# ducha-aiki/affnet

Measured on NVIDIA H100. Metric: Mpix/s end-to-end HesAffNet(+OriNet)+HardNet, higher is better.
Workload: dtype fp16 operands (fp16 residual planes: AffNet/OriNet weights+activations, HardNet layer 2-3 weights), fp32 accumulate; stencils fp32

## Files before the change

affnet_b200/csrc/nets_tcx.cu:

```cuda
#include <stdlib.h>
#include <string.h>

#include <vector>

#include <cuda_bf16.h>

#include "net_impl.cuh"
#include "tcx_conv.cuh"
#include "tcx_first.cuh"

namespace ag {
namespace tcx {

static int num_sms() {
    static int n = 0;
    if (n == 0) {
        int dev = 0;
        cudaGetDevice(&dev);
        cudaDeviceGetAttribute(&n, cudaDevAttrMultiProcessorCount, dev);
        if (n <= 0) n = 132;
    }
    return n;
}

static int ensure_smem_attr(const void* func, int bytes, bool* configured, const char* what) {
    int dev = 0;
    cudaGetDevice(&dev);
    dev &= 63;
    if (configured[dev]) return AG_OK;
    int rc = check_cuda(cudaFuncSetAttribute(func, cudaFuncAttributeMaxDynamicSharedMemorySize, bytes), what);
    if (rc == AG_OK) configured[dev] = true;
    return rc;
}

template <int CIN, int COUT, int H, int STRIDE, int NSPLIT, int STAGES, int OUT, int SA, int SW, int OSA, int BF = 0, int MC = 0>
static int launch_conv(const void* in, void* out, const __half* w, const float* b, float inv_scale, int n, int group, const int* count, cudaStream_t st) {
    using Cfg = XCfg<CIN, COUT, H, STRIDE, NSPLIT, STAGES, OUT, SA, SW, OSA>;
    auto kern = tcx_conv_kernel<CIN, COUT, H, STRIDE, NSPLIT, STAGES, OUT, SA, SW, OSA, BF, MC>;
    static bool configured[64] = {};
    int rc = ensure_smem_attr((const void*)kern, (int)Cfg::SMEM, configured, "tcx_conv smem attr");
    if (rc != AG_OK) return rc;
    XArgs a;
    a.in = (const __half*)in; a.out = out; a.wpk = w; a.bias = b; a.inv_scale = inv_scale; a.n = n; a.group = group; a.count = count;
    const int units = Cfg::In::PAIR ? (n + 1) / 2 : n;
    int gx = num_sms() / NSPLIT;
    if (gx > units) gx = units;
    if (gx < 1) gx = 1;
    if (MC) {
        cudaLaunchConfig_t cfg;
        memset(&cfg, 0, sizeof(cfg));
        cfg.gridDim = dim3(gx, NSPLIT); cfg.blockDim = dim3(Cfg::THREADS); cfg.dynamicSmemBytes = Cfg::SMEM; cfg.stream = st;
        cudaLaunchAttribute attr[1];
        attr[0].id = cudaLaunchAttributeClusterDimension;
        attr[0].val.clusterDim.x = 1; attr[0].val.clusterDim.y = 2; attr[0].val.clusterDim.z = 1;
        cfg.attrs = attr; cfg.numAttrs = 1;
        rc = check_cuda(cudaLaunchKernelEx(&cfg, kern, a), "tcx_conv cluster launch");
        if (rc != AG_OK) return rc;
    } else
        kern<<<dim3(gx, NSPLIT), Cfg::THREADS, Cfg::SMEM, st>>>(a);
    AG_CHECK_LAUNCH("tcx_conv_kernel");
    return AG_OK;
}

template <int C1, int COUT, int SA, int SW, int OSA, int BF = 0, int L3 = 0>
static int launch_first(void* out, const __half* w, const float* b, float inv_scale, int n, int group, const int* count, cudaStream_t st, const FirstSrc& src,
                        void* out3 = nullptr, const __half* w3 = nullptr, const float* b3 = nullptr, float inv_scale3 = 0.f) {
    using Cfg = XFirstCfg<C1, COUT, SA, SW, OSA, L3>;
    auto kern = tcx_first_kernel<C1, COUT, SA, SW, OSA, BF, L3>;
    static bool configured[64] = {};
    int rc = ensure_smem_attr((const void*)kern, (int)Cfg::SMEM, configured, "tcx_first smem attr");
    if (rc != AG_OK) return rc;
    XArgs a;
    a.in = nullptr; a.out = out; a.wpk = w; a.bias = b; a.inv_scale = inv_scale; a.n = n; a.group = group; a.count = count;
    XArgs a3 = a;
    a3.out = out3; a3.wpk = w3; a3.bias = b3; a3.inv_scale = inv_scale3;
    int gx = num_sms();
    if (gx > n) gx = n;
    if (gx < 1) gx = 1;
    kern<<<gx, Cfg::THREADS, Cfg::SMEM, st>>>(a, src, a3);
    AG_CHECK_LAUNCH("tcx_first_kernel");
    return AG_OK;
}

__global__ void tcx_decode_kernel(const __half* __restrict__ buf, int layout, int C, int osa, int H, int n, float* __restrict__ out) {
    const size_t total = (size_t)n * C * H * H;
    for (size_t i = (size_t)blockIdx.x * blockDim.x + threadIdx.x; i < total; i += (size_t)gridDim.x * blockDim.x) {
        const int x = (int)(i % H), y = (int)((i / H) % H), c = (int)((i / ((size_t)H * H)) % C), pi = (int)(i / ((size_t)H * H * C));
        const int slots = layout_slots(layout);
        const size_t unit_halfs = (size_t)(C / 8) * slots * 8 * (osa ? 2 : 1);
        const int unit = layout_pair(layout) ? (pi >> 1) : pi;
        const int slot = layout_slot(layout, y, x, pi & 1);
        const __half* ub = buf + (size_t)unit * unit_halfs;
        float v = __half2float(ub[((size_t)(c / 8) * slots + slot) * 8 + (c & 7)]);
        if (osa) v += __half2float(ub[((size_t)(C / 8 + c / 8) * slots + slot) * 8 + (c & 7)]);
        out[i] = v;
    }
}

}

static __half bf16_bits_as_half(float v) {
    const __nv_bfloat16 b = __float2bfloat16_rn(v);
    __half h;
    memcpy(&h, &b, 2);
    return h;
}
static float bf16_round(float v) { return __bfloat162float(__float2bfloat16_rn(v)); }

void tcx_pack_layer(const float* wf, int ci, int co, int stride, int nsplit, int sw, float scale, std::vector<__half>& out, int bf16) {
    const int nt = co / nsplit;
    auto put = [&](int dy, int dx, int cin, int c, int part) {
        const float v = scale * wf[((size_t)(dy * 3 + dx) * ci + cin) * co + c];
        if (bf16) {
            const float hi = bf16_round(v);
            out.push_back(bf16_bits_as_half(part == 0 ? hi : v - hi));
        } else {
            const __half hi = __float2half_rn(v);
            out.push_back(part == 0 ? hi : __float2half_rn(v - __half2float(hi)));
        }
    };
    for (int sp = 0; sp < nsplit; sp++)
        for (int dy = 0; dy < 3; dy++)
            for (int j = 0; j < ci / 16; j++) {
                if (stride == 1) {
                    for (int kg = 0; kg < 2; kg++)
                        for (int part = 0; part <= sw; part++)
                            for (int dx = 0; dx < 3; dx++)
                                for (int c = 0; c < nt; c++)
                                    for (int e = 0; e < 8; e++) put(dy, dx, (2 * j + kg) * 8 + e, sp * nt + c, part);
                } else {
                    for (int kg = 0; kg < 2; kg++)
                        for (int part = 0; part <= sw; part++)
                            for (int dx = 0; dx < 3; dx += 2)
                                for (int c = 0; c < nt; c++)
                                    for (int e = 0; e < 8; e++) put(dy, dx, (2 * j + kg) * 8 + e, sp * nt + c, part);
                    for (int kg = 0; kg < 2; kg++)
                        for (int part = 0; part <= sw; part++)
                            for (int c = 0; c < nt; c++)
                                for (int e = 0; e < 8; e++) put(dy, 1, (2 * j + kg) * 8 + e, sp * nt + c, part);
                }
            }
}

int tcx_nsplit(int kind, int layer) { return (kind == AG_NET_HARDNET && layer >= 4) ? 2 : 1; }
#ifndef AG_HARD_SW2
#define AG_HARD_SW2 1
#endif
#ifndef AG_HARD_SW3
#define AG_HARD_SW3 1
#endif
#ifndef AG_HARD_SW4
#define AG_HARD_SW4 0
#endif
int tcx_split_w(int kind, int layer) { return kind == AG_NET_HARDNET ? (layer == 1 ? AG_HARD_SW2 : layer == 2 ? AG_HARD_SW3 : layer == 3 ? AG_HARD_SW4 : 0) : 1; }
int tcx_stride(int layer) { return (layer == 2 || layer == 4) ? 2 : 1; }

size_t tcx_act_bytes(int n) { return (size_t)(n + 1) * 65536; }

#ifndef AG_HARD_MC5
#define AG_HARD_MC5 1
#endif
#ifndef AG_HARD_MC6
#define AG_HARD_MC6 0
#endif
int tcx_trunk_affori(const ag_net* net, const tc::FirstSrc& src0, int n, int group, const int* count, void* bufA, void* bufB, void* feat,
                     cudaStream_t st, int upto) {
    using namespace tcx;
    tc::FirstSrc src = src0;
    src.w1 = net->d_w1; src.b1 = net->d_b[0]; src.w1_inv = net->w_inv_scale[0]; src.w1_scale = 1.0f / net->w_inv_scale[0];
    int rc;
    if (upto <= 2) return launch_first<16, 16, 1, 1, 1>(bufB, net->d_wx[1], net->d_b[1], net->w_inv_scale[1], n, group, count, st, src);
    if ((rc = launch_first<16, 16, 1, 1, 1, 0, 1>(nullptr, net->d_wx[1], net->d_b[1], net->w_inv_scale[1], n, group, count, st, src,
                                                   bufA, net->d_wx[2], net->d_b[2], net->w_inv_scale[2]))) return rc;
    if (upto <= 3) return AG_OK;
    if ((rc = launch_conv<32, 32, 16, 1, 1, 4, L_S2_8P, 1, 1, 1>(bufA, bufB, net->d_wx[3], net->d_b[3], net->w_inv_scale[3], n, group, count, st))) return rc;
    if (upto <= 4) return AG_OK;
    if ((rc = launch_conv<32, 64, 16, 2, 1, 2, L_S1_8P, 1, 1, 1>(bufB, bufA, net->d_wx[4], net->d_b[4], net->w_inv_scale[4], n, group, count, st))) return rc;
    if (upto <= 5) return AG_OK;
    return launch_conv<64, 64, 8, 1, 1, 2, L_HEAD, 1, 1, 1>(bufA, feat, net->d_wx[5], net->d_b[5], net->w_inv_scale[5], n, group, count, st);
}

template <int BF>
static int trunk_hardnet_t(const ag_net* net, const tc::FirstSrc& src0, int n, int group, const int* count, void* bufA, void* bufB, void* headbuf,
                           cudaStream_t st, int upto) {
    using namespace tcx;
    tc::FirstSrc src = src0;
    src.w1 = net->d_w1; src.b1 = net->d_b[0]; src.w1_inv = net->w_inv_scale[0]; src.w1_scale = 1.0f / net->w_inv_scale[0];
    __half* const* wx = BF ? net->d_wx_bf : net->d_wx;
    int rc;
    if ((rc = launch_first<32, 32, 0, AG_HARD_SW2, 0, BF>(bufB, wx[1], net->d_b[1], net->w_inv_scale[1], n, group, count, st, src))) return rc;
    if (upto <= 2) return AG_OK;
    if ((rc = launch_conv<32, 64, 32, 2, 1, 2, L_S1_16, 0, AG_HARD_SW3, 0, BF>(bufB, bufA, wx[2], net->d_b[2], net->w_inv_scale[2], n, group, count, st))) return rc;
    if (upto <= 3) return AG_OK;
    if ((rc = launch_conv<64, 64, 16, 1, 1, 2, L_S2_8P, 0, AG_HARD_SW4, 0, BF>(bufA, bufB, wx[3], net->d_b[3], net->w_inv_scale[3], n, group, count, st))) return rc;
    if (upto <= 4) return AG_OK;
    if ((rc = launch_conv<64, 128, 16, 2, 2, 2, L_S1_8P, 0, 0, 0, BF, AG_HARD_MC5>(bufB, bufA, wx[4], net->d_b[4], net->w_inv_scale[4], n, group, count, st))) return rc;
    if (upto <= 5) return AG_OK;
    return launch_conv<128, 128, 8, 1, 2, 2, L_HEAD, 0, 0, 0, BF, AG_HARD_MC6>(bufA, headbuf, wx[5], net->d_b[5], net->w_inv_scale[5], n, group, count, st);
}

int tcx_trunk_hardnet(const ag_net* net, const tc::FirstSrc& src0, int n, int group, const int* count, void* bufA, void* bufB, void* headbuf,
                      cudaStream_t st, int upto, int bf16) {
    return bf16 ? trunk_hardnet_t<1>(net, src0, n, group, count, bufA, bufB, headbuf, st, upto)
                : trunk_hardnet_t<0>(net, src0, n, group, count, bufA, bufB, headbuf, st, upto);
}

}

using namespace ag;

extern "C" {

int ag_debug_tcx_layer(const ag_net_t* net, const float* d_patches, int n, int upto, float* d_out, void* d_ws, size_t ws_bytes, void* stream) {
    AG_REQUIRE(net && d_patches && d_out && d_ws, "NULL argument");
    AG_REQUIRE(upto >= 2 && upto <= 5 && n >= 1, "layer out of range");
    const size_t act = align_up(tcx_act_bytes(n), 256);
    AG_REQUIRE(ws_bytes >= 2 * act, "workspace too small");
    cudaStream_t st = (cudaStream_t)stream;
    char* base = (char*)d_ws;
    const tc::FirstSrc src = tc_src_patches(d_patches);
    const bool hard = net->kind == AG_NET_HARDNET;
    int rc = hard ? tcx_trunk_hardnet(net, src, n, n, nullptr, base, base + act, nullptr, st, upto)
                  : tcx_trunk_affori(net, src, n, n, nullptr, base, base + act, nullptr, st, upto);
    if (rc) return rc;
    const int lay = upto == 2 ? tcx::L_S2_16 : upto == 3 ? tcx::L_S1_16 : upto == 4 ? tcx::L_S2_8P : tcx::L_S1_8P;
    const int H = upto == 2 ? 32 : (upto <= 4 ? 16 : 8);
    const int Cb = hard ? 32 : 16;
    const int C = upto == 2 ? Cb : (upto <= 4 ? 2 * Cb : 4 * Cb);
    const void* buf = (upto == 2 || upto == 4) ? base + act : base;
    const int osa = hard ? 0 : 1;
    tcx::tcx_decode_kernel<<<296, 256, 0, st>>>((const __half*)buf, lay, C, osa, H, n, d_out);
    AG_CHECK_LAUNCH("tcx_decode_kernel");
    return AG_OK;
}

#ifdef AG_FIRST_TIMELINE
int ag_first_timeline_read(unsigned long long* host, int* dims, int reset) {
    constexpr size_t n = (size_t)tcx::TL_LAUNCHES * tcx::TL_CTAS * 16 * tcx::TL_STATES;
    if (dims) { dims[0] = tcx::TL_LAUNCHES; dims[1] = tcx::TL_CTAS; dims[2] = tcx::TL_STATES; }
    cudaDeviceSynchronize();
    if (host) {
        const int rc = check_cuda(cudaMemcpyFromSymbol(host, tcx::g_first_tl, n * 8), "timeline read");
        if (rc != AG_OK) return rc;
    }
    if (reset) {
        static unsigned long long zeros[n];
        static int zl[tcx::TL_CTAS];
        int rc = check_cuda(cudaMemcpyToSymbol(tcx::g_first_tl, zeros, sizeof(zeros)), "timeline reset");
        if (rc == AG_OK) rc = check_cuda(cudaMemcpyToSymbol(tcx::g_first_tl_launch, zl, sizeof(zl)), "timeline reset");
        return rc;
    }
    return AG_OK;
}
#endif

}
```

affnet_b200/csrc/tcx_conv.cuh:

```cuda
#pragma once
#include <cuda_bf16.h>

#include "tc_conv.cuh"

namespace ag {
namespace tcx {

using namespace ag::tc;

enum XLayout { L_S2_16 = 0, L_S1_16 = 1, L_S2_8P = 2, L_S1_8P = 3, L_HEAD = 4 };

__device__ __forceinline__ void bulk_g2s_mc(void* dst, const void* src, uint32_t bytes, uint64_t* bar, uint16_t mask) {
    asm volatile("cp.async.bulk.shared::cluster.global.mbarrier::complete_tx::bytes.multicast::cluster [%0], [%1], %2, [%3], %4;" ::"r"(smem_u32(dst)),
                 "l"(src), "r"(bytes), "r"(smem_u32(bar)), "h"(mask)
                 : "memory");
}
__device__ __forceinline__ void mbar_arrive_cluster(uint64_t* bar, uint32_t cta) {
    asm volatile("{\n .reg .b32 ra;\n mapa.shared::cluster.u32 ra, %0, %1;\n mbarrier.arrive.release.cluster.shared::cluster.b64 _, [ra];\n}\n" ::"r"(smem_u32(bar)), "r"(cta)
                 : "memory");
}
__device__ __forceinline__ void cluster_sync() {
    asm volatile("barrier.cluster.arrive.release.aligned;\n barrier.cluster.wait.acquire.aligned;" ::: "memory");
}

template <int BF>
__device__ __forceinline__ uint32_t pack2(float a, float b) {
    if (BF) { const __nv_bfloat162 h = __floats2bfloat162_rn(a, b); return *reinterpret_cast<const uint32_t*>(&h); }
    const __half2 h = __floats2half2_rn(a, b);
    return *reinterpret_cast<const uint32_t*>(&h);
}
template <int BF>
__device__ __forceinline__ float2 unpack2(uint32_t u) {
    if (BF) return make_float2(__uint_as_float(u << 16), __uint_as_float(u & 0xFFFF0000u));
    return __half22float2(*reinterpret_cast<const __half2*>(&u));
}
template <int LO, int BF = 0>
__device__ __forceinline__ void split_pack8(const float* v, uint4& hi, uint4& lo) {
    uint32_t h[4], l[4];
#pragma unroll
    for (int i = 0; i < 4; i++) {
        h[i] = pack2<BF>(v[2 * i], v[2 * i + 1]);
        if (LO) {
            const float2 f = unpack2<BF>(h[i]);
            l[i] = pack2<BF>(v[2 * i] - f.x, v[2 * i + 1] - f.y);
        } else l[i] = 0;
    }
    hi = make_uint4(h[0], h[1], h[2], h[3]);
    lo = make_uint4(l[0], l[1], l[2], l[3]);
}

template <int LO, int BF = 0>
__device__ __forceinline__ void split_pack2(float v0, float v1, uint32_t& hi, uint32_t& lo) {
    hi = pack2<BF>(v0, v1);
    if (LO) {
        const float2 f = unpack2<BF>(hi);
        lo = pack2<BF>(v0 - f.x, v1 - f.y);
    } else lo = 0;
}

__host__ __device__ constexpr int layout_slots(int lay) { return lay == L_S2_16 ? 1024 : lay == L_S1_16 ? 256 : lay == L_S2_8P ? 512 : 128; }
__host__ __device__ constexpr int layout_pair(int lay) { return (lay == L_S2_8P || lay == L_S1_8P) ? 1 : 0; }
__host__ __device__ constexpr int layout_slot(int lay, int y, int x, int p) {
    return lay == L_S2_16 ? ((y & 1) * 2 + (x & 1)) * 256 + (y >> 1) * 16 + (x >> 1)
         : lay == L_S1_16 ? y * 16 + x
         : lay == L_S2_8P ? ((y & 1) * 2 + (x & 1)) * 128 + ((y >> 1) * 2 + p) * 8 + (x >> 1)
                          : (y * 2 + p) * 8 + x;
}

template <int H, int STRIDE>
struct XIn {
    static constexpr int HOUT = H / STRIDE;
    static constexpr int PAIR = (HOUT == 8) ? 1 : 0;
    static constexpr int W = HOUT;
    static constexpr int RW = W * (1 + PAIR);
    static constexpr int TILES = HOUT * RW / 128;
    static constexpr int NPLANES = (STRIDE == 1) ? 1 : 4;
    static constexpr int DATA = HOUT * RW;
    static constexpr int PLANE = DATA + RW;
    static constexpr int SLOT_STAGE = NPLANES * PLANE;
    static constexpr int LAYOUT = (STRIDE == 2) ? (PAIR ? L_S2_8P : L_S2_16) : (PAIR ? L_S1_8P : L_S1_16);
    static_assert(HOUT == 8 || HOUT == 16 || HOUT == 32, "map sizes of the three nets");
    static_assert(!(STRIDE == 1 && H == 32), "the 32x32 stride-1 layer lives in tcx_first.cuh");
};

struct XArgs {
    const __half* in;
    void* out;
    const __half* wpk;
    const float* bias;
    float inv_scale;
    int n, group;
    const int* count;
};

template <int CIN, int COUT, int H, int STRIDE, int NSPLIT, int STAGES, int OUT, int SA, int SW, int OSA>
struct XCfg {
    using In = XIn<H, STRIDE>;
    static constexpr int CO = COUT, STRD = STRIDE, OUTL = OUT, SPLIT_A = SA, SPLIT_W = SW, SPLIT_O = OSA;
    static constexpr int KC = CIN / 8, NT = COUT / NSPLIT, HOUT = In::HOUT;
    static constexpr int G = KC * (1 + SA);
    static constexpr int GS = STAGES * In::SLOT_STAGE + (STRIDE == 1 ? In::RW : 0);
    static constexpr int ACCW = 3 * NT;
    static constexpr int BLOCKS = 2 * In::TILES;
    static constexpr uint32_t W_BYTES = 9u * CIN * NT * 2u * (1 + SW);
    static constexpr uint32_t IN_BYTES = (uint32_t)G * GS * 16u;
    static constexpr uint32_t HI_IN_BYTES = (uint32_t)KC * In::NPLANES * In::DATA * 16u;
    static constexpr uint32_t UNIT_IN_BYTES = HI_IN_BYTES * (1 + SA);
    static constexpr int THREADS = 288;
    static constexpr size_t SMEM = 1024 + (size_t)W_BYTES + IN_BYTES;
    static constexpr size_t HI_OUT_BYTES = (size_t)(COUT / 8) * layout_slots(OUT) * 16;
    static constexpr size_t UNIT_OUT_BYTES = (OUT == L_HEAD) ? 0 : HI_OUT_BYTES * (1 + OSA);
    static constexpr int NR1 = (1 + SW) * 3 * NT;
    static constexpr int NRO = (1 + SW) * 2 * NT, NRE = (1 + SW) * NT;
    static_assert(CIN % 16 == 0 && NT % 16 == 0 && ACCW <= 256, "wgmma shape");
    static_assert(In::W == 8 || In::W == 16, "a warp's 16 accumulator rows hold whole image rows");
    static_assert(SA <= 1 && SW <= 1 && OSA <= 1, "split-precision switches are 0 | 1");
    static_assert(2 * STAGES + 1 <= 60, "barrier area");
    static_assert(SMEM <= 232448, "shared memory budget");
    static_assert(GS < 16384, "leading-byte offset field");
    static_assert(OUT == L_HEAD || layout_pair(OUT) || !In::PAIR, "a pair layer writes pair layouts or the head operand");
};

__device__ __forceinline__ void frag_left(float v0, float v1, int lane, float& l0, float& l1) {
    const float s0 = __shfl_sync(0xffffffffu, v0, (lane + 28) & 31), s1 = __shfl_sync(0xffffffffu, v1, (lane + 28) & 31);
    l0 = s0;
    l1 = lane < 4 ? s0 : s1;
}
__device__ __forceinline__ void frag_right(float v0, float v1, int lane, float& r0, float& r1) {
    const float t0 = __shfl_sync(0xffffffffu, v0, (lane + 4) & 31), t1 = __shfl_sync(0xffffffffu, v1, (lane + 4) & 31);
    r0 = lane >= 28 ? t1 : t0;
    r1 = t1;
}

__device__ __forceinline__ bool xpatch_valid(const XArgs& a, int pi) { return pi < a.n && (a.count == nullptr || (pi % a.group) < a.count[pi / a.group]); }

template <class Cfg, int BF>
__device__ __forceinline__ void xconv_block_issue(float* d, uint32_t a_t, uint32_t w_base) {
    using In = typename Cfg::In;
    constexpr int KC = Cfg::KC, NT = Cfg::NT, GS = Cfg::GS, RW = In::RW, SA = Cfg::SPLIT_A, SW = Cfg::SPLIT_W;
    constexpr uint32_t LBO_A = ((uint32_t)GS) << 16;
    wgmma_fence();
    if (Cfg::STRD == 1) {
#pragma unroll
        for (int dy = 0; dy < 3; dy++) {
#pragma unroll
            for (int j = 0; j < KC / 2; j++) {
                const uint32_t ahi = ((a_t + (uint32_t)(dy * RW + 2 * j * GS)) & 0x3FFFu) | LBO_A;
                const uint32_t alo = ((a_t + (uint32_t)(dy * RW + (KC + 2 * j) * GS)) & 0x3FFFu) | LBO_A;
                const uint32_t blk = w_base + (uint32_t)((dy * (KC / 2) + j) * 2 * Cfg::NR1);
                const uint32_t bhi = (blk & 0x3FFFu) | ((uint32_t)Cfg::NR1 << 16), blo = ((blk + 3 * NT) & 0x3FFFu) | ((uint32_t)Cfg::NR1 << 16);
                Wgmma<3 * NT, BF>::mma(d, desc64(ahi), desc64(bhi), (dy | j) != 0);
                if (SW) Wgmma<3 * NT, BF>::mma(d, desc64(ahi), desc64(blo), 1);
                if (SA) Wgmma<3 * NT, BF>::mma(d, desc64(alo), desc64(bhi), 1);
            }
        }
    } else {
#pragma unroll
        for (int dy = 0; dy < 3; dy++) {
            constexpr int PL = In::PLANE;
            const int py = (dy == 1) ? 0 : 1, ro = (dy == 0) ? 0 : 1;
#pragma unroll
            for (int j = 0; j < KC / 2; j++) {
                const uint32_t blk = w_base + (uint32_t)((dy * (KC / 2) + j) * 2 * (Cfg::NRO + Cfg::NRE));
                const uint32_t bo_hi = (blk & 0x3FFFu) | ((uint32_t)Cfg::NRO << 16), bo_lo = ((blk + 2 * NT) & 0x3FFFu) | ((uint32_t)Cfg::NRO << 16);
                const uint32_t be = blk + 2 * Cfg::NRO;
                const uint32_t be_hi = (be & 0x3FFFu) | ((uint32_t)Cfg::NRE << 16), be_lo = ((be + NT) & 0x3FFFu) | ((uint32_t)Cfg::NRE << 16);
                const uint32_t ao = a_t + (uint32_t)((py * 2 + 1) * PL + ro * RW);
                const uint32_t ao_hi = ((ao + (uint32_t)(2 * j * GS)) & 0x3FFFu) | LBO_A, ao_lo = ((ao + (uint32_t)((KC + 2 * j) * GS)) & 0x3FFFu) | LBO_A;
                Wgmma<2 * NT, BF>::mma(d, desc64(ao_hi), desc64(bo_hi), (dy | j) != 0);
                if (SW) Wgmma<2 * NT, BF>::mma(d, desc64(ao_hi), desc64(bo_lo), 1);
                if (SA) Wgmma<2 * NT, BF>::mma(d, desc64(ao_lo), desc64(bo_hi), 1);
                const uint32_t ae = a_t + (uint32_t)((py * 2 + 0) * PL + ro * RW);
                const uint32_t ae_hi = ((ae + (uint32_t)(2 * j * GS)) & 0x3FFFu) | LBO_A, ae_lo = ((ae + (uint32_t)((KC + 2 * j) * GS)) & 0x3FFFu) | LBO_A;
                Wgmma<NT, BF>::mma(d + NT, desc64(ae_hi), desc64(be_hi), (dy | j) != 0);
                if (SW) Wgmma<NT, BF>::mma(d + NT, desc64(ae_hi), desc64(be_lo), 1);
                if (SA) Wgmma<NT, BF>::mma(d + NT, desc64(ae_lo), desc64(be_hi), 1);
            }
        }
    }
    wgmma_commit();
}
template <class Cfg, int BF>
__device__ __forceinline__ void xconv_block_mma(float* d, uint32_t a_t, uint32_t w_base) {
    xconv_block_issue<Cfg, BF>(d, a_t, w_base);
    wgmma_wait<0>();
    wgmma_reg_fence<Cfg::ACCW / 2>(d);
}

template <class Cfg, int BF>
__device__ __forceinline__ void xconv_block_epilogue(const float* d, const XArgs& a, const float* s_bias, int u, int b, int split, int wq, int lane) {
    using In = typename Cfg::In;
    constexpr int NT = Cfg::NT, HOUT = Cfg::HOUT, W = In::W, PAIR = In::PAIR, COUT = Cfg::CO, OUT = Cfg::OUTL, OSA = Cfg::SPLIT_O;
    unsigned char* obase[2];
    bool has_l[2], has_r[2];
    bool ok[2];
    size_t lo_off = 0;
#pragma unroll
    for (int h = 0; h < 2; h++) {
        const int r = b * 64 + wq * 16 + (lane >> 2) + 8 * h;
        int y, x, pi;
        if (PAIR) { y = r >> 4; x = r & 7; pi = 2 * u + ((r >> 3) & 1); }
        else { y = r / W; x = r - y * W; pi = u; }
        ok[h] = xpatch_valid(a, pi);
        has_l[h] = x > 0; has_r[h] = x < W - 1;
        if (OUT == L_HEAD) {
            obase[h] = reinterpret_cast<unsigned char*>(a.out) + (((size_t)(pi >> 7) * (HOUT * HOUT * COUT / 8) + (size_t)(y * HOUT + x) * (COUT / 8)) * 128 + (pi & 127)) * 16;
            lo_off = (size_t)((a.n + 127) >> 7) * (HOUT * HOUT * COUT / 8) * 128 * 16;
        } else {
            const int ou = layout_pair(OUT) ? (pi >> 1) : pi;
            obase[h] = reinterpret_cast<unsigned char*>(a.out) + (size_t)ou * Cfg::UNIT_OUT_BYTES + (size_t)layout_slot(OUT, y, x, pi & 1) * 16;
            lo_off = (size_t)(COUT / 8) * layout_slots(OUT) * 16;
        }
    }
#pragma unroll
    for (int j = 0; j < NT / 8; j++) {
        const int c = j * 8 + 2 * (lane & 3);
        float v[2][2];
#pragma unroll
        for (int e = 0; e < 2; e++) {
            const float c00 = d[4 * j + e], c01 = d[4 * j + 2 + e];
            const float c10 = d[4 * (j + NT / 8) + e], c11 = d[4 * (j + NT / 8) + 2 + e];
            const float c20 = d[4 * (j + 2 * NT / 8) + e], c21 = d[4 * (j + 2 * NT / 8) + 2 + e];
            float l0, l1;
            frag_left(c00, c01, lane, l0, l1);
            float acc0, acc1;
            if (Cfg::STRD == 1) {
                float r0, r1;
                frag_right(c20, c21, lane, r0, r1);
                const float t0 = has_r[0] ? r0 + c10 : c10, t1 = has_r[1] ? r1 + c11 : c11;
                acc0 = has_l[0] ? l0 + t0 : t0;
                acc1 = has_l[1] ? l1 + t1 : t1;
            } else {
                const float t0 = c10 + c20, t1 = c11 + c21;
                acc0 = has_l[0] ? l0 + t0 : t0;
                acc1 = has_l[1] ? l1 + t1 : t1;
            }
            v[0][e] = fmaxf(fmaf(acc0, a.inv_scale, s_bias[c + e]), 0.f);
            v[1][e] = fmaxf(fmaf(acc1, a.inv_scale, s_bias[c + e]), 0.f);
        }
        const int ch = split * NT + c;
        const size_t goff = ((OUT == L_HEAD) ? (size_t)(ch / 8) * 128 * 16 : (size_t)(ch / 8) * layout_slots(OUT) * 16) + (ch & 7) * 2;
#pragma unroll
        for (int h = 0; h < 2; h++) {
            if (!ok[h]) continue;
            uint32_t hi, lo;
            split_pack2<OSA, BF>(v[h][0], v[h][1], hi, lo);
            *reinterpret_cast<uint32_t*>(obase[h] + goff) = hi;
            if (OSA) *reinterpret_cast<uint32_t*>(obase[h] + lo_off + goff) = lo;
        }
    }
}

template <int CIN, int COUT, int H, int STRIDE, int NSPLIT, int STAGES, int OUT, int SA, int SW, int OSA, int BF = 0, int MC = 0>
__global__ void __launch_bounds__(288, 1) tcx_conv_kernel(const XArgs a) {
    static_assert(MC == 0 || NSPLIT == 2, "multicast pairs the two channel-split CTAs");
    using Cfg = XCfg<CIN, COUT, H, STRIDE, NSPLIT, STAGES, OUT, SA, SW, OSA>;
    using In = typename Cfg::In;
    constexpr int ACCW = Cfg::ACCW, BLOCKS = Cfg::BLOCKS, GS = Cfg::GS, RW = In::RW;
    constexpr int PAIR = In::PAIR;
    extern __shared__ __align__(1024) unsigned char smem[];
    uint64_t* full = reinterpret_cast<uint64_t*>(smem);
    uint64_t* empty = full + STAGES;
    uint64_t* wbar = empty + STAGES;
    float* s_bias = reinterpret_cast<float*>(smem + 512);
    unsigned char* sW = smem + 1024;
    unsigned char* sIn = sW + Cfg::W_BYTES;

    const int warp = threadIdx.x >> 5, lane = threadIdx.x & 31;
    const int split = blockIdx.y;
    const int n_units = PAIR ? (a.n + 1) >> 1 : a.n;

    if (threadIdx.x < Cfg::NT) s_bias[threadIdx.x] = a.bias[split * Cfg::NT + threadIdx.x];
    if (threadIdx.x == 0) {
        for (int s = 0; s < STAGES; s++) { mbar_init(&full[s], 1); mbar_init(&empty[s], 2 * (1 + MC)); }
        mbar_init(wbar, 1);
        asm volatile("fence.mbarrier_init.release.cluster;" ::: "memory");
    }
    for (int i = threadIdx.x; i < (int)(Cfg::IN_BYTES / 16); i += blockDim.x) reinterpret_cast<uint4*>(sIn)[i] = make_uint4(0, 0, 0, 0);
    asm volatile("fence.proxy.async.shared::cta;" ::: "memory");
    __syncthreads();
    if (MC) cluster_sync();

    auto uvalid = [&](int u) -> bool { return PAIR ? (xpatch_valid(a, 2 * u) || xpatch_valid(a, 2 * u + 1)) : xpatch_valid(a, u); };

    if (warp == 8) {
        if (lane == 0) {
            mbar_expect_tx(wbar, Cfg::W_BYTES);
            bulk_g2s(sW, reinterpret_cast<const unsigned char*>(a.wpk) + (size_t)split * Cfg::W_BYTES, Cfg::W_BYTES, wbar);
            int it = 0;
            for (int u = blockIdx.x; u < n_units; u += gridDim.x) {
                if (!uvalid(u)) continue;
                const int s = it % STAGES;
                mbar_wait(&empty[s], ((it / STAGES) & 1) ^ 1);
                mbar_expect_tx(&full[s], Cfg::UNIT_IN_BYTES);
                const unsigned char* gsrc = reinterpret_cast<const unsigned char*>(a.in) + (size_t)u * Cfg::UNIT_IN_BYTES;
#pragma unroll 1
                for (int g = 0; g < Cfg::G; g++)
#pragma unroll
                    for (int pl = 0; pl < In::NPLANES; pl++) {
                        unsigned char* dst = sIn + ((size_t)g * GS + (size_t)s * In::SLOT_STAGE + (size_t)pl * In::PLANE + RW) * 16;
                        const unsigned char* srcp = gsrc + ((size_t)g * In::NPLANES + pl) * In::DATA * 16;
                        if (MC) { if (((g * In::NPLANES + pl) & 1) == split) bulk_g2s_mc(dst, srcp, In::DATA * 16u, &full[s], (uint16_t)3); }
                        else bulk_g2s(dst, srcp, In::DATA * 16u, &full[s]);
                    }
                it++;
            }
            if (MC) {
                for (int k = 0; k < STAGES && k < it; k++) { const int j = it - 1 - k; mbar_wait(&empty[j % STAGES], (j / STAGES) & 1); }
            }
        }
    } else if (warp < 8) {
        const int wg = warp >> 2, wq = warp & 3;
        mbar_wait(wbar, 0);
        const uint32_t w_base = smem_u32(sW) >> 4;
        const uint32_t in_base = smem_u32(sIn) >> 4;
        int it = 0;
        for (int u = blockIdx.x; u < n_units; u += gridDim.x) {
            if (!uvalid(u)) continue;
            const int s = it % STAGES;
            mbar_wait(&full[s], (it / STAGES) & 1);
            const uint32_t st_base = in_base + (uint32_t)(s * In::SLOT_STAGE);
#pragma unroll 1
            for (int b = wg; b < BLOCKS; b += 2) {
                float d[ACCW / 2];
                xconv_block_mma<Cfg, BF>(d, st_base + (uint32_t)(b * 64), w_base);
                xconv_block_epilogue<Cfg, BF>(d, a, s_bias, u, b, split, wq, lane);
            }
            bar_sync(3 + wg, 128);
            if ((threadIdx.x & 127) == 0) {
                if (MC) { mbar_arrive_cluster(&empty[s], 0); mbar_arrive_cluster(&empty[s], 1); }
                else mbar_arrive(&empty[s]);
            }
            it++;
        }
    }
    __syncthreads();
    if (MC) cluster_sync();
}

}
}
```

Before: 473.8.

## Double-buffer wgmma accumulators to overlap epilogue with next block's MMA in pair stride-1 convs

For pair-layout stride-1 conv layers, the consumer warpgroups now keep two accumulator sets and issue the next block's wgmma before running the current block's epilogue, so tensor-core work overlaps the bias/ReLU/store epilogue. To fit two accumulators the kernel grows to 384 threads and uses setmaxnreg to move registers from the loader warpgroup to the consumers. The stage-release barrier is moved ahead of the epilogue. Optional clock64 timeline instrumentation is also added behind a compile-time macro. The change raises register pressure and risks spills or reduced overlap if the epilogue dominates.

```diff
diff --git a/affnet_b200/csrc/nets_tcx.cu b/affnet_b200/csrc/nets_tcx.cu
--- a/affnet_b200/csrc/nets_tcx.cu
+++ b/affnet_b200/csrc/nets_tcx.cu
@@ -254,4 +254,24 @@
 }
 #endif
 
-}
+#ifdef AG_CONV_TIMELINE
+int ag_conv_timeline_read(unsigned long long* host, int* dims, int reset) {
+    constexpr size_t n = (size_t)tcx::CTL_LAUNCHES * tcx::CTL_CTAS * tcx::CTL_WARPS * tcx::CTL_STATES;
+    if (dims) { dims[0] = tcx::CTL_LAUNCHES; dims[1] = tcx::CTL_CTAS; dims[2] = tcx::CTL_WARPS; dims[3] = tcx::CTL_STATES; }
+    cudaDeviceSynchronize();
+    if (host) {
+        const int rc = check_cuda(cudaMemcpyFromSymbol(host, tcx::g_conv_tl, n * 8), "timeline read");
+        if (rc != AG_OK) return rc;
+    }
+    if (reset) {
+        static unsigned long long zeros[n];
+        static int zl[tcx::CTL_CTAS];
+        int rc = check_cuda(cudaMemcpyToSymbol(tcx::g_conv_tl, zeros, sizeof(zeros)), "timeline reset");
+        if (rc == AG_OK) rc = check_cuda(cudaMemcpyToSymbol(tcx::g_conv_tl_launch, zl, sizeof(zl)), "timeline reset");
+        return rc;
+    }
+    return AG_OK;
+}
+#endif
+
+}
diff --git a/affnet_b200/csrc/tcx_conv.cuh b/affnet_b200/csrc/tcx_conv.cuh
--- a/affnet_b200/csrc/tcx_conv.cuh
+++ b/affnet_b200/csrc/tcx_conv.cuh
@@ -3,10 +3,23 @@
 
 #include "tc_conv.cuh"
 
+#ifdef AG_CONV_TIMELINE
+#define AG_CTL(state, ...) do { const long long t_ = clock64(); __VA_ARGS__; ctl[state] += (unsigned long long)(clock64() - t_); } while (0)
+#else
+#define AG_CTL(state, ...) do { __VA_ARGS__; } while (0)
+#endif
+
 namespace ag {
 namespace tcx {
 
 using namespace ag::tc;
+
+enum { CTL_TOTAL, CTL_WAIT_FULL, CTL_ISSUE, CTL_MMA_WAIT, CTL_WG_BAR, CTL_EPILOGUE, CTL_WAIT_EMPTY, CTL_COPY, CTL_STATES };
+#ifdef AG_CONV_TIMELINE
+constexpr int CTL_CTAS = 4, CTL_LAUNCHES = 12, CTL_WARPS = 12;
+__device__ unsigned long long g_conv_tl[CTL_LAUNCHES][CTL_CTAS][CTL_WARPS][CTL_STATES];
+__device__ int g_conv_tl_launch[CTL_CTAS];
+#endif
 
 enum XLayout { L_S2_16 = 0, L_S1_16 = 1, L_S2_8P = 2, L_S1_8P = 3, L_HEAD = 4 };
 
@@ -106,7 +119,10 @@
     static constexpr uint32_t IN_BYTES = (uint32_t)G * GS * 16u;
     static constexpr uint32_t HI_IN_BYTES = (uint32_t)KC * In::NPLANES * In::DATA * 16u;
     static constexpr uint32_t UNIT_IN_BYTES = HI_IN_BYTES * (1 + SA);
-    static constexpr int THREADS = 288;
+    static constexpr int PIPE = (In::PAIR && STRIDE == 1) ? 1 : 0;
+    static constexpr int THREADS = PIPE ? 384 : 288;
+    static constexpr int REG_LOADER = 40, REG_CONSUMER = 232;
+    static_assert(128 * REG_LOADER + 256 * REG_CONSUMER <= 65536 && REG_LOADER % 8 == 0 && REG_CONSUMER % 8 == 0, "register split");
     static constexpr size_t SMEM = 1024 + (size_t)W_BYTES + IN_BYTES;
     static constexpr size_t HI_OUT_BYTES = (size_t)(COUT / 8) * layout_slots(OUT) * 16;
     static constexpr size_t UNIT_OUT_BYTES = (OUT == L_HEAD) ? 0 : HI_OUT_BYTES * (1 + OSA);
@@ -180,13 +196,6 @@
     }
     wgmma_commit();
 }
-template <class Cfg, int BF>
-__device__ __forceinline__ void xconv_block_mma(float* d, uint32_t a_t, uint32_t w_base) {
-    xconv_block_issue<Cfg, BF>(d, a_t, w_base);
-    wgmma_wait<0>();
-    wgmma_reg_fence<Cfg::ACCW / 2>(d);
-}
-
 template <class Cfg, int BF>
 __device__ __forceinline__ void xconv_block_epilogue(const float* d, const XArgs& a, const float* s_bias, int u, int b, int split, int wq, int lane) {
     using In = typename Cfg::In;
@@ -252,7 +261,7 @@
 }
 
 template <int CIN, int COUT, int H, int STRIDE, int NSPLIT, int STAGES, int OUT, int SA, int SW, int OSA, int BF = 0, int MC = 0>
-__global__ void __launch_bounds__(288, 1) tcx_conv_kernel(const XArgs a) {
+__global__ void __launch_bounds__(XCfg<CIN, COUT, H, STRIDE, NSPLIT, STAGES, OUT, SA, SW, OSA>::THREADS, 1) tcx_conv_kernel(const XArgs a) {
     static_assert(MC == 0 || NSPLIT == 2, "multicast pairs the two channel-split CTAs");
     using Cfg = XCfg<CIN, COUT, H, STRIDE, NSPLIT, STAGES, OUT, SA, SW, OSA>;
     using In = typename Cfg::In;
@@ -277,21 +286,34 @@
         asm volatile("fence.mbarrier_init.release.cluster;" ::: "memory");
     }
     for (int i = threadIdx.x; i < (int)(Cfg::IN_BYTES / 16); i += blockDim.x) reinterpret_cast<uint4*>(sIn)[i] = make_uint4(0, 0, 0, 0);
+#ifdef AG_CONV_TIMELINE
+    int* s_tl_slot = reinterpret_cast<int*>(smem + 504);
+    if (threadIdx.x == 0)
+        *s_tl_slot = (blockIdx.x < CTL_CTAS && blockIdx.y == 0) ? min(atomicAdd(&g_conv_tl_launch[blockIdx.x], 1), CTL_LAUNCHES) : CTL_LAUNCHES;
+    unsigned long long ctl[CTL_STATES] = {};
+#endif
     asm volatile("fence.proxy.async.shared::cta;" ::: "memory");
     __syncthreads();
     if (MC) cluster_sync();
+#ifdef AG_CONV_TIMELINE
+    const long long tl_start = clock64();
+#endif
 
     auto uvalid = [&](int u) -> bool { return PAIR ? (xpatch_valid(a, 2 * u) || xpatch_valid(a, 2 * u + 1)) : xpatch_valid(a, u); };
 
-    if (warp == 8) {
-        if (lane == 0) {
+    if (Cfg::PIPE ? warp >= 8 : warp == 8) {
+        if constexpr (Cfg::PIPE) asm volatile("setmaxnreg.dec.sync.aligned.u32 %0;" ::"n"(Cfg::REG_LOADER));
+        if (warp == 8 && lane == 0) {
             mbar_expect_tx(wbar, Cfg::W_BYTES);
             bulk_g2s(sW, reinterpret_cast<const unsigned char*>(a.wpk) + (size_t)split * Cfg::W_BYTES, Cfg::W_BYTES, wbar);
             int it = 0;
             for (int u = blockIdx.x; u < n_units; u += gridDim.x) {
                 if (!uvalid(u)) continue;
                 const int s = it % STAGES;
-                mbar_wait(&empty[s], ((it / STAGES) & 1) ^ 1);
+                AG_CTL(CTL_WAIT_EMPTY, mbar_wait(&empty[s], ((it / STAGES) & 1) ^ 1));
+#ifdef AG_CONV_TIMELINE
+                const long long tc = clock64();
+#endif
                 mbar_expect_tx(&full[s], Cfg::UNIT_IN_BYTES);
                 const unsigned char* gsrc = reinterpret_cast<const unsigned char*>(a.in) + (size_t)u * Cfg::UNIT_IN_BYTES;
 #pragma unroll 1
@@ -303,13 +325,16 @@
                         if (MC) { if (((g * In::NPLANES + pl) & 1) == split) bulk_g2s_mc(dst, srcp, In::DATA * 16u, &full[s], (uint16_t)3); }
                         else bulk_g2s(dst, srcp, In::DATA * 16u, &full[s]);
                     }
+#ifdef AG_CONV_TIMELINE
+                ctl[CTL_COPY] += (unsigned long long)(clock64() - tc);
+#endif
                 it++;
             }
             if (MC) {
                 for (int k = 0; k < STAGES && k < it; k++) { const int j = it - 1 - k; mbar_wait(&empty[j % STAGES], (j / STAGES) & 1); }
             }
         }
-    } else if (warp < 8) {
+    } else if (!Cfg::PIPE && warp < 8) {
         const int wg = warp >> 2, wq = warp & 3;
         mbar_wait(wbar, 0);
         const uint32_t w_base = smem_u32(sW) >> 4;
@@ -318,22 +343,86 @@
         for (int u = blockIdx.x; u < n_units; u += gridDim.x) {
             if (!uvalid(u)) continue;
             const int s = it % STAGES;
-            mbar_wait(&full[s], (it / STAGES) & 1);
+            AG_CTL(CTL_WAIT_FULL, mbar_wait(&full[s], (it / STAGES) & 1));
             const uint32_t st_base = in_base + (uint32_t)(s * In::SLOT_STAGE);
 #pragma unroll 1
             for (int b = wg; b < BLOCKS; b += 2) {
                 float d[ACCW / 2];
-                xconv_block_mma<Cfg, BF>(d, st_base + (uint32_t)(b * 64), w_base);
-                xconv_block_epilogue<Cfg, BF>(d, a, s_bias, u, b, split, wq, lane);
-            }
-            bar_sync(3 + wg, 128);
+                AG_CTL(CTL_ISSUE, xconv_block_issue<Cfg, BF>(d, st_base + (uint32_t)(b * 64), w_base));
+                AG_CTL(CTL_MMA_WAIT, wgmma_wait<0>());
+                wgmma_reg_fence<ACCW / 2>(d);
+                AG_CTL(CTL_EPILOGUE, xconv_block_epilogue<Cfg, BF>(d, a, s_bias, u, b, split, wq, lane));
+            }
+            AG_CTL(CTL_WG_BAR, bar_sync(3 + wg, 128));
             if ((threadIdx.x & 127) == 0) {
                 if (MC) { mbar_arrive_cluster(&empty[s], 0); mbar_arrive_cluster(&empty[s], 1); }
                 else mbar_arrive(&empty[s]);
             }
             it++;
         }
-    }
+    } else if constexpr (Cfg::PIPE) {
+        asm volatile("setmaxnreg.inc.sync.aligned.u32 %0;" ::"n"(Cfg::REG_CONSUMER));
+        const int wg = warp >> 2, wq = warp & 3;
+        mbar_wait(wbar, 0);
+        const uint32_t w_base = smem_u32(sW) >> 4;
+        const uint32_t in_base = smem_u32(sIn) >> 4;
+        struct Job { int u, it, b; };
+        auto next_unit = [&](int u) -> int {
+            do u += gridDim.x; while (u < n_units && !uvalid(u));
+            return u;
+        };
+        auto advance = [&](Job j) -> Job {
+            j.b += 2;
+            if (j.b >= BLOCKS) { j.b = wg; j.u = next_unit(j.u); j.it++; }
+            return j;
+        };
+        auto issue = [&](float* d, const Job& j) {
+            const int s = j.it % STAGES;
+            if (j.b == wg) AG_CTL(CTL_WAIT_FULL, mbar_wait(&full[s], (j.it / STAGES) & 1));
+            uint32_t wb = w_base;
+            asm volatile("" : "+r"(wb));
+            AG_CTL(CTL_ISSUE, xconv_block_issue<Cfg, BF>(d, in_base + (uint32_t)(s * In::SLOT_STAGE + j.b * 64), wb));
+        };
+        auto finish = [&](float* d, const Job& j) {
+            wgmma_reg_fence<ACCW / 2>(d);
+            if (j.b + 2 >= BLOCKS) {
+                AG_CTL(CTL_WG_BAR, bar_sync(3 + wg, 128));
+                if ((threadIdx.x & 127) == 0) {
+                    const int s = j.it % STAGES;
+                    if (MC) { mbar_arrive_cluster(&empty[s], 0); mbar_arrive_cluster(&empty[s], 1); }
+                    else mbar_arrive(&empty[s]);
+                }
+            }
+            int ln = lane, sp = split;
+            asm volatile("" : "+r"(ln), "+r"(sp));
+            AG_CTL(CTL_EPILOGUE, xconv_block_epilogue<Cfg, BF>(d, a, s_bias, j.u, j.b, sp, wq, ln));
+        };
+        Job cur{(int)blockIdx.x, 0, wg};
+        if (cur.u < n_units && !uvalid(cur.u)) cur.u = next_unit(cur.u);
+        if (cur.u < n_units) {
+            float d0[ACCW / 2], d1[ACCW / 2];
+            issue(d0, cur);
+            while (true) {
+                Job nx = advance(cur);
+                if (nx.u >= n_units) { AG_CTL(CTL_MMA_WAIT, wgmma_wait<0>()); finish(d0, cur); break; }
+                issue(d1, nx);
+                AG_CTL(CTL_MMA_WAIT, wgmma_wait<1>());
+                finish(d0, cur);
+                cur = nx;
+                nx = advance(cur);
+                if (nx.u >= n_units) { AG_CTL(CTL_MMA_WAIT, wgmma_wait<0>()); finish(d1, cur); break; }
+                issue(d0, nx);
+                AG_CTL(CTL_MMA_WAIT, wgmma_wait<1>());
+                finish(d1, cur);
+                cur = nx;
+            }
+        }
+    }
+#ifdef AG_CONV_TIMELINE
+    ctl[CTL_TOTAL] = (unsigned long long)(clock64() - tl_start);
+    if (lane == 0 && *s_tl_slot < CTL_LAUNCHES)
+        for (int i = 0; i < CTL_STATES; i++) g_conv_tl[*s_tl_slot][blockIdx.x][warp][i] = ctl[i];
+#endif
     __syncthreads();
     if (MC) cluster_sync();
 }
```

New measurement: 480.5 (median of 6 runs). 1.4% higher.

## Add ping-pong warpgroup MMA scheduling and early stage release in conv kernel

Applied to the files above, without the earlier changes.

Adds a ping-pong schedule between the two consumer warpgroups: named barriers make them take turns issuing wgmma, so one warpgroup's epilogue overlaps the other's MMA. The input stage is now released per warp right after the last block's MMA completes, before the epilogue, replacing the warpgroup barrier plus single arrive. Empty-barrier arrival counts change to match, and the cluster arrive is relaxed to release.cta scope. It is enabled only for the head layers and HardNet layer 5, and adds optional clock64 timeline instrumentation behind a compile flag. The risks are serialising MMA issue between warpgroups and a memory-ordering hazard from the weaker arrive scope.

```diff
diff --git a/affnet_b200/csrc/nets_tcx.cu b/affnet_b200/csrc/nets_tcx.cu
--- a/affnet_b200/csrc/nets_tcx.cu
+++ b/affnet_b200/csrc/nets_tcx.cu
@@ -33,10 +33,10 @@
     return rc;
 }
 
-template <int CIN, int COUT, int H, int STRIDE, int NSPLIT, int STAGES, int OUT, int SA, int SW, int OSA, int BF = 0, int MC = 0>
+template <int CIN, int COUT, int H, int STRIDE, int NSPLIT, int STAGES, int OUT, int SA, int SW, int OSA, int BF = 0, int MC = 0, int PPS = 0>
 static int launch_conv(const void* in, void* out, const __half* w, const float* b, float inv_scale, int n, int group, const int* count, cudaStream_t st) {
     using Cfg = XCfg<CIN, COUT, H, STRIDE, NSPLIT, STAGES, OUT, SA, SW, OSA>;
-    auto kern = tcx_conv_kernel<CIN, COUT, H, STRIDE, NSPLIT, STAGES, OUT, SA, SW, OSA, BF, MC>;
+    auto kern = tcx_conv_kernel<CIN, COUT, H, STRIDE, NSPLIT, STAGES, OUT, SA, SW, OSA, BF, MC, PPS>;
     static bool configured[64] = {};
     int rc = ensure_smem_attr((const void*)kern, (int)Cfg::SMEM, configured, "tcx_conv smem attr");
     if (rc != AG_OK) return rc;
@@ -177,7 +177,7 @@
     if (upto <= 4) return AG_OK;
     if ((rc = launch_conv<32, 64, 16, 2, 1, 2, L_S1_8P, 1, 1, 1>(bufB, bufA, net->d_wx[4], net->d_b[4], net->w_inv_scale[4], n, group, count, st))) return rc;
     if (upto <= 5) return AG_OK;
-    return launch_conv<64, 64, 8, 1, 1, 2, L_HEAD, 1, 1, 1>(bufA, feat, net->d_wx[5], net->d_b[5], net->w_inv_scale[5], n, group, count, st);
+    return launch_conv<64, 64, 8, 1, 1, 2, L_HEAD, 1, 1, 1, 0, 0, 1>(bufA, feat, net->d_wx[5], net->d_b[5], net->w_inv_scale[5], n, group, count, st);
 }
 
 template <int BF>
@@ -194,9 +194,9 @@
     if (upto <= 3) return AG_OK;
     if ((rc = launch_conv<64, 64, 16, 1, 1, 2, L_S2_8P, 0, AG_HARD_SW4, 0, BF>(bufA, bufB, wx[3], net->d_b[3], net->w_inv_scale[3], n, group, count, st))) return rc;
     if (upto <= 4) return AG_OK;
-    if ((rc = launch_conv<64, 128, 16, 2, 2, 2, L_S1_8P, 0, 0, 0, BF, AG_HARD_MC5>(bufB, bufA, wx[4], net->d_b[4], net->w_inv_scale[4], n, group, count, st))) return rc;
+    if ((rc = launch_conv<64, 128, 16, 2, 2, 2, L_S1_8P, 0, 0, 0, BF, AG_HARD_MC5, 1>(bufB, bufA, wx[4], net->d_b[4], net->w_inv_scale[4], n, group, count, st))) return rc;
     if (upto <= 5) return AG_OK;
-    return launch_conv<128, 128, 8, 1, 2, 2, L_HEAD, 0, 0, 0, BF, AG_HARD_MC6>(bufA, headbuf, wx[5], net->d_b[5], net->w_inv_scale[5], n, group, count, st);
+    return launch_conv<128, 128, 8, 1, 2, 2, L_HEAD, 0, 0, 0, BF, AG_HARD_MC6, 1>(bufA, headbuf, wx[5], net->d_b[5], net->w_inv_scale[5], n, group, count, st);
 }
 
 int tcx_trunk_hardnet(const ag_net* net, const tc::FirstSrc& src0, int n, int group, const int* count, void* bufA, void* bufB, void* headbuf,
@@ -254,4 +254,25 @@
 }
 #endif
 
-}
+#ifdef AG_CONV_TIMELINE
+int ag_conv_timeline_read(unsigned long long* sums, unsigned long long* events, int* dims, int reset) {
+    using namespace tcx;
+    if (dims) { dims[0] = CT_LAUNCHES; dims[1] = CT_CTAS; dims[2] = CT_STATES; dims[3] = CT_EVENTS; }
+    int rc = check_cuda(cudaDeviceSynchronize(), "timeline read");
+    if (rc == AG_OK && sums) rc = check_cuda(cudaMemcpyFromSymbol(sums, g_conv_tl, sizeof(g_conv_tl)), "timeline read");
+    if (rc == AG_OK && events) rc = check_cuda(cudaMemcpyFromSymbol(events, g_conv_ev, sizeof(g_conv_ev)), "timeline read");
+    if (rc == AG_OK && reset) {
+        void* p = nullptr;
+        const int zl[CT_CTAS] = {};
+        if (rc == AG_OK) rc = check_cuda(cudaGetSymbolAddress(&p, g_conv_tl), "timeline reset");
+        if (rc == AG_OK) rc = check_cuda(cudaMemset(p, 0, sizeof(g_conv_tl)), "timeline reset");
+        if (rc == AG_OK) rc = check_cuda(cudaGetSymbolAddress(&p, g_conv_ev), "timeline reset");
+        if (rc == AG_OK) rc = check_cuda(cudaMemset(p, 0, sizeof(g_conv_ev)), "timeline reset");
+        if (rc == AG_OK) rc = check_cuda(cudaMemcpyToSymbol(g_conv_tl_launch, zl, sizeof(zl)), "timeline reset");
+        if (rc == AG_OK) rc = check_cuda(cudaDeviceSynchronize(), "timeline reset");
+    }
+    return rc;
+}
+#endif
+
+}
diff --git a/affnet_b200/csrc/tcx_conv.cuh b/affnet_b200/csrc/tcx_conv.cuh
--- a/affnet_b200/csrc/tcx_conv.cuh
+++ b/affnet_b200/csrc/tcx_conv.cuh
@@ -3,10 +3,56 @@
 
 #include "tc_conv.cuh"
 
+#ifndef AG_CONV_PINGPONG
+#define AG_CONV_PINGPONG 1
+#endif
+
 namespace ag {
 namespace tcx {
 
 using namespace ag::tc;
+
+constexpr int XORDER = 5;
+
+enum { CT_TOTAL, CT_WAIT_FULL, CT_TURN, CT_ISSUE, CT_MMA_WAIT, CT_EPILOGUE, CT_WG_BAR, CT_WAIT_EMPTY, CT_OTHER, CT_STATES };
+#ifdef AG_CONV_TIMELINE
+constexpr int CT_CTAS = 4, CT_LAUNCHES = 16, CT_EVENTS = 2048;
+__device__ unsigned long long g_conv_tl[CT_LAUNCHES][CT_CTAS][9][CT_STATES];
+__device__ unsigned long long g_conv_ev[CT_LAUNCHES][2][CT_EVENTS][3];
+__device__ int g_conv_tl_launch[CT_CTAS];
+struct ConvTimeline {
+    unsigned long long t[CT_STATES];
+    long long start, mark;
+    int slot, warp, n_ev;
+    __device__ static void claim(int* s_slot) {
+        if (threadIdx.x == 0)
+            *s_slot = (blockIdx.y == 0 && blockIdx.x < CT_CTAS) ? min(atomicAdd(&g_conv_tl_launch[blockIdx.x], 1), CT_LAUNCHES) : CT_LAUNCHES;
+    }
+    __device__ void init(const int* s_slot) {
+        for (int i = 0; i < CT_STATES; i++) t[i] = 0;
+        slot = *s_slot; warp = threadIdx.x >> 5; n_ev = 0;
+        start = mark = clock64();
+    }
+    __device__ void lap(int state) { const long long now = clock64(); t[state] += (unsigned long long)(now - mark); mark = now; }
+    __device__ void event(int k) {
+        if (blockIdx.x == 0 && slot < CT_LAUNCHES && (threadIdx.x & 127) == 0 && n_ev < CT_EVENTS) g_conv_ev[slot][warp >> 2][n_ev][k] = (unsigned long long)mark;
+        if (k == 2) n_ev++;
+    }
+    __device__ void finish() {
+        t[CT_TOTAL] = (unsigned long long)(clock64() - start);
+        if ((threadIdx.x & 31) == 0 && slot < CT_LAUNCHES)
+            for (int i = 0; i < CT_STATES; i++) g_conv_tl[slot][blockIdx.x][warp][i] = t[i];
+    }
+};
+#else
+struct ConvTimeline {
+    __device__ static void claim(int*) {}
+    __device__ void init(const int*) {}
+    __device__ void lap(int) {}
+    __device__ void event(int) {}
+    __device__ void finish() {}
+};
+#endif
 
 enum XLayout { L_S2_16 = 0, L_S1_16 = 1, L_S2_8P = 2, L_S1_8P = 3, L_HEAD = 4 };
 
@@ -16,7 +62,7 @@
                  : "memory");
 }
 __device__ __forceinline__ void mbar_arrive_cluster(uint64_t* bar, uint32_t cta) {
-    asm volatile("{\n .reg .b32 ra;\n mapa.shared::cluster.u32 ra, %0, %1;\n mbarrier.arrive.release.cluster.shared::cluster.b64 _, [ra];\n}\n" ::"r"(smem_u32(bar)), "r"(cta)
+    asm volatile("{\n .reg .b32 ra;\n mapa.shared::cluster.u32 ra, %0, %1;\n mbarrier.arrive.release.cta.shared::cluster.b64 _, [ra];\n}\n" ::"r"(smem_u32(bar)), "r"(cta)
                  : "memory");
 }
 __device__ __forceinline__ void cluster_sync() {
@@ -181,13 +227,6 @@
     wgmma_commit();
 }
 template <class Cfg, int BF>
-__device__ __forceinline__ void xconv_block_mma(float* d, uint32_t a_t, uint32_t w_base) {
-    xconv_block_issue<Cfg, BF>(d, a_t, w_base);
-    wgmma_wait<0>();
-    wgmma_reg_fence<Cfg::ACCW / 2>(d);
-}
-
-template <class Cfg, int BF>
 __device__ __forceinline__ void xconv_block_epilogue(const float* d, const XArgs& a, const float* s_bias, int u, int b, int split, int wq, int lane) {
     using In = typename Cfg::In;
     constexpr int NT = Cfg::NT, HOUT = Cfg::HOUT, W = In::W, PAIR = In::PAIR, COUT = Cfg::CO, OUT = Cfg::OUTL, OSA = Cfg::SPLIT_O;
@@ -251,13 +290,14 @@
     }
 }
 
-template <int CIN, int COUT, int H, int STRIDE, int NSPLIT, int STAGES, int OUT, int SA, int SW, int OSA, int BF = 0, int MC = 0>
+template <int CIN, int COUT, int H, int STRIDE, int NSPLIT, int STAGES, int OUT, int SA, int SW, int OSA, int BF = 0, int MC = 0, int PPS = 0>
 __global__ void __launch_bounds__(288, 1) tcx_conv_kernel(const XArgs a) {
     static_assert(MC == 0 || NSPLIT == 2, "multicast pairs the two channel-split CTAs");
     using Cfg = XCfg<CIN, COUT, H, STRIDE, NSPLIT, STAGES, OUT, SA, SW, OSA>;
     using In = typename Cfg::In;
     constexpr int ACCW = Cfg::ACCW, BLOCKS = Cfg::BLOCKS, GS = Cfg::GS, RW = In::RW;
     constexpr int PAIR = In::PAIR;
+    constexpr bool PP = AG_CONV_PINGPONG && PPS;
     extern __shared__ __align__(1024) unsigned char smem[];
     uint64_t* full = reinterpret_cast<uint64_t*>(smem);
     uint64_t* empty = full + STAGES;
@@ -270,16 +310,25 @@
     const int split = blockIdx.y;
     const int n_units = PAIR ? (a.n + 1) >> 1 : a.n;
 
+    int* s_tl_slot = reinterpret_cast<int*>(smem + 496);
+
     if (threadIdx.x < Cfg::NT) s_bias[threadIdx.x] = a.bias[split * Cfg::NT + threadIdx.x];
     if (threadIdx.x == 0) {
-        for (int s = 0; s < STAGES; s++) { mbar_init(&full[s], 1); mbar_init(&empty[s], 2 * (1 + MC)); }
+        for (int s = 0; s < STAGES; s++) { mbar_init(&full[s], 1); mbar_init(&empty[s], (PP ? 8 : 2) * (1 + MC)); }
         mbar_init(wbar, 1);
         asm volatile("fence.mbarrier_init.release.cluster;" ::: "memory");
     }
+    ConvTimeline::claim(s_tl_slot);
     for (int i = threadIdx.x; i < (int)(Cfg::IN_BYTES / 16); i += blockDim.x) reinterpret_cast<uint4*>(sIn)[i] = make_uint4(0, 0, 0, 0);
     asm volatile("fence.proxy.async.shared::cta;" ::: "memory");
     __syncthreads();
     if (MC) cluster_sync();
+    ConvTimeline tl;
+    tl.init(s_tl_slot);
+    auto release = [&](uint64_t* e) {
+        if (MC) { mbar_arrive_cluster(e, 0); mbar_arrive_cluster(e, 1); }
+        else mbar_arrive(e);
+    };
 
     auto uvalid = [&](int u) -> bool { return PAIR ? (xpatch_valid(a, 2 * u) || xpatch_valid(a, 2 * u + 1)) : xpatch_valid(a, u); };
 
@@ -291,7 +340,9 @@
             for (int u = blockIdx.x; u < n_units; u += gridDim.x) {
                 if (!uvalid(u)) continue;
                 const int s = it % STAGES;
+                tl.lap(CT_OTHER);
                 mbar_wait(&empty[s], ((it / STAGES) & 1) ^ 1);
+                tl.lap(CT_WAIT_EMPTY);
                 mbar_expect_tx(&full[s], Cfg::UNIT_IN_BYTES);
                 const unsigned char* gsrc = reinterpret_cast<const unsigned char*>(a.in) + (size_t)u * Cfg::UNIT_IN_BYTES;
 #pragma unroll 1
@@ -305,9 +356,11 @@
                     }
                 it++;
             }
+            tl.lap(CT_OTHER);
             if (MC) {
                 for (int k = 0; k < STAGES && k < it; k++) { const int j = it - 1 - k; mbar_wait(&empty[j % STAGES], (j / STAGES) & 1); }
             }
+            tl.lap(CT_WAIT_EMPTY);
         }
     } else if (warp < 8) {
         const int wg = warp >> 2, wq = warp & 3;
@@ -318,22 +371,39 @@
         for (int u = blockIdx.x; u < n_units; u += gridDim.x) {
             if (!uvalid(u)) continue;
             const int s = it % STAGES;
+            tl.lap(CT_OTHER);
             mbar_wait(&full[s], (it / STAGES) & 1);
+            tl.lap(CT_WAIT_FULL);
             const uint32_t st_base = in_base + (uint32_t)(s * In::SLOT_STAGE);
 #pragma unroll 1
             for (int b = wg; b < BLOCKS; b += 2) {
                 float d[ACCW / 2];
-                xconv_block_mma<Cfg, BF>(d, st_base + (uint32_t)(b * 64), w_base);
+                if (PP && (wg == 1 || it > 0 || b > 0)) bar_sync(XORDER + wg, 256);
+                tl.lap(CT_TURN);
+                tl.event(0);
+                xconv_block_issue<Cfg, BF>(d, st_base + (uint32_t)(b * 64), w_base);
+                if (PP) asm volatile("bar.arrive %0, 256;" ::"r"(XORDER + (wg ^ 1)) : "memory");
+                tl.lap(CT_ISSUE);
+                wgmma_wait<0>();
+                wgmma_reg_fence<ACCW / 2>(d);
+                tl.lap(CT_MMA_WAIT);
+                tl.event(1);
+                if (PP && b + 2 >= BLOCKS && lane == 0) release(&empty[s]);
                 xconv_block_epilogue<Cfg, BF>(d, a, s_bias, u, b, split, wq, lane);
-            }
-            bar_sync(3 + wg, 128);
-            if ((threadIdx.x & 127) == 0) {
-                if (MC) { mbar_arrive_cluster(&empty[s], 0); mbar_arrive_cluster(&empty[s], 1); }
-                else mbar_arrive(&empty[s]);
+                tl.lap(CT_EPILOGUE);
+                tl.event(2);
+            }
+            if (!PP) {
+                bar_sync(3 + wg, 128);
+                tl.lap(CT_WG_BAR);
+                if ((threadIdx.x & 127) == 0) release(&empty[s]);
             }
             it++;
         }
-    }
+        if (PP && wg == 0 && it > 0) bar_sync(XORDER, 256);
+        tl.lap(CT_OTHER);
+    }
+    tl.finish();
     __syncthreads();
     if (MC) cluster_sync();
 }
```

Measured after the change: 473.6 before, 489.9 after (median of 6 runs). 1.03x the previous value.
